# PimLb/POMDP_PBVI_Exploration

Hardware: AMD Instinct MI355X
Metric: alpha-vector backups/sec (higher is better)
Workload: dtype f32

## Files before the change

pomdp_pbvi_exploration_amd/csrc/backup_kernels.h:

```cpp
#pragma once
#include "pbvi_common.h"

namespace pbvi {

template <typename T>
struct ModelView {
    int S, S_pad, A, O, R;
    const int32_t* rs;
    const T* rto;
    const T* er;
    const uint8_t* sup;
};

__host__ __device__ __forceinline__ int64_t push_row_index(int o, int a, int b, int A, int B) {
#ifdef PBVI_PUSH_ORDER_OAB
    return ((int64_t)o * A + a) * B + b;
#else
    return ((int64_t)o * B + b) * A + a;
#endif
}

template <typename T>
struct SlabView {
    const T* slabs;
// ... 48 lines not shown
                             int k_tiles, uint8_t* need, hipStream_t st);

template <typename T>
hipError_t launch_dead(const T* bel, int ldb, int B, ModelView<T> mv,
                       const unsigned long long* nzBw ,
                       int k_tiles, uint8_t* dead, int32_t* btl ,
                       int32_t* btc , int* dead_count ,
                       hipStream_t st, const uint8_t* rowflags = nullptr ,
                       const int32_t* perm = nullptr );

template <typename T>
hipError_t launch_push_project(const T* bel, int ldb, int B, ModelView<T> mv, const int32_t* in_ptr,
                               const int32_t* in_src, double gamma, const T* amax, T* bp, int ldp, double* mag,
                               hipStream_t st, uint8_t* nzP = nullptr );
template <typename T>
hipError_t launch_rdot(const T* bel, int ldb, int B, ModelView<T> mv, const int32_t* btl, const int32_t* btc, double* rd,
                       hipStream_t st);

template <typename T>
hipError_t launch_argmax(SlabView<T> sv, int V, int G, int B, const uint8_t* dead, double tol_rel, double tol_abs,
                         const int* chain_steps ,
                         int flag_all, int32_t* best_v, double* best_score, double* err, int32_t* queue, int* qcount,
                         hipStream_t st, double tol_extra = 0.0 ,
                         int split = 0 );

template <typename T>
hipError_t launch_fold_chunk(SlabView<T> sv, int B, int G, int Vc, int V, int v0, int tail_cols, T* dst, int64_t ldd,
                             const int* chain, int* chain_max, hipStream_t st);

struct RefineWork {
    int32_t* items_v = nullptr;
    int32_t* items_slot = nullptr;
    double* scores = nullptr;
    int32_t* slot_entry = nullptr;
    int32_t* slot_n = nullptr;
    int32_t* tiles = nullptr;
    unsigned long long* emax = nullptr;
    int32_t* eidx = nullptr;
    double* ib_val = nullptr;
    int32_t* ib_idx = nullptr;
    int* cnt = nullptr;
    int32_t* q2_entry = nullptr;
    int32_t* q2_n = nullptr;
    int32_t* q2_cand = nullptr;
    double* q2_part = nullptr;
    int* q2_done = nullptr;
    int q2_cap = 0;
// ... 6 lines not shown
    uint8_t* nzW = nullptr;
    int* klistW = nullptr;
    int* kcountW = nullptr;
    const int32_t* in_ptr = nullptr;
    const int32_t* in_src = nullptr;
    const float* gam = nullptr;
    int ldg = 0;
    double l1_rel = 0.0;
};

template <typename T, typename TS>
hipError_t launch_refine(bool proj, SlabView<TS> sv, int V, int G, int max_entries, const int32_t* queue,
                         const int* qcount, const T* bel, int ldb, const T* alpha, int lda, ModelView<T> mv,
                         double gamma, const int32_t* btl, const int32_t* btc ,
                         const uint8_t* nzG ,
                         int32_t* best_v, double* best_score, double* err, int* cand_total ,
                         RefineWork work, hipStream_t st);

template <typename T, typename TS>
hipError_t launch_refine_scan(bool proj, SlabView<TS> sv, int V, int G, int max_entries, const int32_t* queue,
                              const int* qcount, const T* bel, int ldb, const T* alpha, int lda, ModelView<T> mv,
                              double gamma, const int32_t* btl, const int32_t* btc, const uint8_t* nzG, int32_t* best_v,
                              double* best_score, double* err, int* cand_total, RefineWork work, int* counts_host,
                              hipStream_t st);
template <typename T>
hipError_t launch_refine_deferred(bool proj, int V, int G, const T* bel, int ldb, const T* alpha, int lda, ModelView<T> mv,
                                  double gamma, int32_t* best_v, double* best_score, double* err, RefineWork work,
                                  int h_items, int h_slots, hipStream_t st);

template <typename T>
hipError_t launch_belief_tiles(const T* bel, int ldb, int B, int S, int k_tiles, int32_t* btl, int32_t* btc,
                               hipStream_t st);

template <typename T>
hipError_t launch_tail_rows(ModelView<T> mv, T* gam , int64_t row0 , int ldg, hipStream_t st,
                            const int32_t* ctile = nullptr);
template <typename T>
hipError_t launch_action(int B, ModelView<T> mv, SlabView<T> sv, int64_t rd_col0, double tol_rel, const int* chain_steps,
                         const double* best_score, const double* err, double* rdot, double* rdot_err, int32_t* action,
                         int32_t* aqueue, int* aqcount, hipStream_t st, double tol_extra = 0.0,
                         uint8_t* acand = nullptr ,
                         int split = 0 );
constexpr int ACTION_SPLIT = 8;
template <typename T>
hipError_t launch_refine_action(const T* bel, int ldb, int B, const T* alpha, int lda, ModelView<T> mv, double gamma,
                                const int32_t* btl, const int32_t* btc, const int32_t* aqueue, const int* aqcount,
                                const double* rdot, const double* rdot_err, const int32_t* best_v,
// ... 38 lines not shown
```

pomdp_pbvi_exploration_amd/csrc/backup_kernels.hip:

```cpp
#include "backup_kernels.h"

#include <cstdlib>
#include <limits>

namespace pbvi {

__device__ __forceinline__ double wave_sum(double v) {
#pragma unroll
    for (int off = 32; off > 0; off >>= 1) v += __shfl_xor(v, off, 64);
    return v;
}

__device__ __forceinline__ double block_sum(double v, double* sh) {
    v = wave_sum(v);
    const int lane = threadIdx.x & 63, wid = threadIdx.x >> 6;
    __syncthreads();
    if (lane == 0) sh[wid] = v;
    __syncthreads();
    return ((sh[0] + sh[1]) + sh[2]) + sh[3];
}

struct TileList {
    const int32_t* list;
    int count;
// ... 556 lines not shown
    return hipGetLastError();
}

template <typename T>
hipError_t launch_dead(const T* bel, int ldb, int B, ModelView<T> mv, const unsigned long long* nzBw, int k_tiles, uint8_t* dead,
                       int32_t* btl, int32_t* btc, int* dead_count, hipStream_t st, const uint8_t* rowflags,
                       const int32_t* perm) {
    if (B <= 0) return hipSuccess;
    const size_t lds = (size_t)((k_tiles + 7) & ~7) + (size_t)((k_tiles + 63) / 64) * 8;
    hipLaunchKernelGGL(k_dead<T>, dim3(B), dim3(256), lds, st, bel, ldb, mv, nzBw, k_tiles, dead, btl, btc,
                       dead_count, rowflags, perm);
    return hipGetLastError();
}

__device__ __forceinline__ double score_window(double tol_rel, const int* chain_steps, int split) {
    const double u24 = 5.9604644775390625e-08;
    double tr = tol_rel;
    if (chain_steps != nullptr && tol_rel < 0.0)
        tr = 8.0 * u24 * (sqrt((double)chain_steps[0] * 32.0 * (split ? 3.0 : 1.0)) + 1.0);
    if (split) tr = (tr + 3.1 * 1.52587890625e-05) * (1.0 + 4.8828125e-04);
    return tr;
}

template <typename T>
__global__ void k_argmax(SlabView<T> sv, int V, int G, int B, const uint8_t* __restrict__ dead, double tol_rel,
                         double tol_abs, double tol_extra, const int* __restrict__ chain_steps, int flag_all, int32_t* __restrict__ best_v, double* __restrict__ best_score,
                         double* __restrict__ err, int32_t* __restrict__ queue, int* __restrict__ qcount, int split) {
    const int lane = threadIdx.x & 63;
    const int64_t gw = (int64_t)blockIdx.x * 4 + (threadIdx.x >> 6);
    if (gw >= (int64_t)B * G) return;
    const int b = (int)(gw / G), g = (int)(gw % G);
    if (dead != nullptr && dead[gw]) {
        if (lane == 0) {
            best_v[gw] = 0;
            best_score[gw] = 0.0;
            err[gw] = 0.0;
        }
        return;
    }
    T m = -std::numeric_limits<T>::infinity(), m2 = -std::numeric_limits<T>::infinity();
    int idx = 0x7fffffff;
    bool vec4 = false;
    if constexpr (sizeof(T) == 4) vec4 = sv.nchunks != nullptr && (sv.push || (V & 3) == 0) && (sv.ldc & 3) == 0;
    if (vec4) {
        typedef float F4 __attribute__((ext_vector_type(4)));
        const int64_t row = sv.push ? sv.push_row(b, g) : (int64_t)b;
        const int64_t col0 = sv.push ? 0 : (int64_t)g * V;
        const float* rowp = (const float*)sv.slabs + row * sv.ldc + col0;
        const int tm = (int)(row >> 8);
        for (int c00 = lane * 4; c00 < V; c00 += 1024) {
            int n[4], fb[4];
            F4 acc[4];
#pragma unroll
            for (int j = 0; j < 4; ++j) {
                const int c0 = c00 + 256 * j;
                const int64_t pair = ((col0 + c0) >> 8) * sv.tiles_m + tm;
                n[j] = c0 < V ? sv.nchunks[pair] : 0;
                fb[j] = (c0 < V && sv.first_block != nullptr) ? sv.first_block[pair] : 0;
            }
#pragma unroll
            for (int j = 0; j < 4; ++j) {
                const F4 zero = {0.f, 0.f, 0.f, 0.f};
                acc[j] = zero;
                if (n[j] > 0) acc[j] = acc[j] + *(const F4*)(rowp + c00 + 256 * j);
            }
#pragma unroll
            for (int j = 0; j < 4; ++j) {
                if (n[j] <= 1) continue;
                if (sv.first_block != nullptr) {
                    const float* x = (const float*)sv.slabs + sv.slab_stride + (int64_t)(fb[j] + 1) * (256 * 256) +
                                     (row & 255) * 256 + ((col0 + c00 + 256 * j) & 255);
                    for (int z = 1; z < n[j]; ++z, x += 256 * 256) acc[j] = acc[j] + *(const F4*)x;
                } else {
                    for (int z = 1; z < n[j]; ++z) acc[j] = acc[j] + *(const F4*)(rowp + c00 + 256 * j + (int64_t)z * sv.slab_stride);
                }
            }
#pragma unroll
            for (int j = 0; j < 4; ++j) {
                const int c0 = c00 + 256 * j;
                if (c0 >= V) break;
#pragma unroll
                for (int i = 0; i < 4; ++i) {
                    const T sc = (T)acc[j][i];
                    const int v = c0 + i;
                    if (v >= V) break;
                    if (sc > m || idx == 0x7fffffff) {
                        m2 = (idx == 0x7fffffff) ? m2 : m;
                        m = sc;
                        idx = v;
                    } else if (sc > m2) {
                        m2 = sc;
                    }
                }
            }
        }
    } else
    for (int v0 = lane; v0 < V; v0 += 256) {
        T sc4[4];
#pragma unroll
        for (int j = 0; j < 4; ++j) {
            const int v = v0 + 64 * j;
            sc4[j] = v < V ? sv.score(b, g, V, v) : T(0);
        }
#pragma unroll
        for (int j = 0; j < 4; ++j) {
            const int v = v0 + 64 * j;
            if (v >= V) break;
            const T sc = sc4[j];
            if (sc > m || idx == 0x7fffffff) {
                m2 = (idx == 0x7fffffff) ? m2 : m;
                m = sc;
                idx = v;
            } else if (sc > m2) {
                m2 = sc;
            }
        }
    }
#pragma unroll
    for (int off = 32; off > 0; off >>= 1) {
        const T om = __shfl_xor(m, off, 64), om2 = __shfl_xor(m2, off, 64);
        const int oi = __shfl_xor(idx, off, 64);
        const T lo = om < m ? om : m;
        T n2 = m2 > om2 ? m2 : om2;
        if (oi != 0x7fffffff && idx != 0x7fffffff) n2 = lo > n2 ? lo : n2;
        if (om > m || (om == m && oi < idx)) {
            m = om;
            idx = oi;
        }
        m2 = n2;
    }
    double E = 0.0;
    int push = 0;
    if (queue != nullptr) {
        const double mag = fmax(fabs((double)m), fabs(sv.magnitude(b, g, G, V)));
        const double tr = score_window(tol_rel, chain_steps, split) + (sv.push ? 2.0 * 5.9604644775390625e-08 : 0.0);
        E = (tr + tol_extra) * mag + tol_abs;
        push = (flag_all || (double)m2 >= (double)m - 2.0 * E) ? 1 : 0;
    }
    if (lane == 0) {
        best_v[gw] = idx;
        best_score[gw] = (double)m;
        err[gw] = E;
        if (push) {
            const int slot = atomicAdd(qcount, 1);
            queue[slot] = (int32_t)gw;
        }
    }
}

template <typename T>
hipError_t launch_argmax(SlabView<T> sv, int V, int G, int B, const uint8_t* dead, double tol_rel, double tol_abs,
                         const int* chain_steps, int flag_all, int32_t* best_v, double* best_score, double* err,
                         int32_t* queue, int* qcount, hipStream_t st, double tol_extra, int split) {
    const int64_t rows = (int64_t)B * G;
    if (rows <= 0) return hipSuccess;
    hipLaunchKernelGGL(k_argmax<T>, dim3((unsigned)((rows + 3) / 4)), dim3(256), 0, st, sv, V, G, B, dead, tol_rel,
                       tol_abs, tol_extra, chain_steps, flag_all, best_v, best_score, err, queue, qcount, split);
    return hipGetLastError();
}

template <typename T>
__global__ void k_fold_chunk(SlabView<T> sv, int B, int G, int Vc, int V, int v0, int tail_cols, T* __restrict__ dst,
                             int64_t ldd, const int* __restrict__ chain, int* __restrict__ chain_max) {
    if (chain != nullptr && blockIdx.x == 0 && blockIdx.y == 0 && threadIdx.x == 0) {
        const int c = chain[0];
        if (c > chain_max[0]) chain_max[0] = c;
    }
    const int64_t group_cols = (int64_t)G * Vc, n_cols = group_cols + tail_cols;
    const int64_t j0 = ((int64_t)blockIdx.x * 256 + threadIdx.x) * 4;
    if (j0 >= n_cols) return;
    bool vec4 = false;
    if constexpr (sizeof(T) == 4) vec4 = sv.nchunks != nullptr && (Vc & 3) == 0 && (sv.ldc & 3) == 0 && j0 + 3 < group_cols;
    auto out_col = [&](int64_t j) -> int64_t {
        if (j >= group_cols) return (int64_t)G * V + (j - group_cols);
        const int64_t g = j / Vc;
        return g * V + v0 + (j - g * Vc);
    };
    const int64_t d0 = out_col(j0);
    for (int b = blockIdx.y; b < B; b += gridDim.y) {
        T* drow = dst + (int64_t)b * ldd;
// ... 72 lines not shown
                for (int j = 0; j < 4; ++j) g[j] += (double)rto[ro + s[j]] * (double)arow[rs[ro + s[j]]];
            }
#pragma unroll
            for (int j = 0; j < 4; ++j) acc[j] += w[j] * ((double)brow[s[j]] * (gamma * g[j]));
        } else {
#pragma unroll
            for (int j = 0; j < 4; ++j) {
                const bool in = s[j] < mv.S;
                acc[j] += (in ? w[j] : 0.0) * ((double)brow[s[j]] * (double)arow[in ? s[j] : 0]);
            }
        }
    }
    return wave_sum((acc[0] + acc[1]) + (acc[2] + acc[3]));
}

template <typename T, typename TS, bool PROJ, bool L1 >
__global__ void k_refine(SlabView<TS> sv, int V, int G, const int32_t* __restrict__ queue,
                         const int* __restrict__ qcount,
                         const T* __restrict__ bel, int ldb, const T* __restrict__ alpha, int lda,
                         ModelView<T> mv, double gamma, const int32_t* __restrict__ btl, const int32_t* __restrict__ btc,
                         const uint8_t* __restrict__ nzG ,
                         int32_t* __restrict__ best_v,
                         double* __restrict__ best_score, double* __restrict__ err, int* __restrict__ cand_total,
                         RefineWork work) {
    __shared__ int cand[256];
    __shared__ int wcount[4];
    __shared__ int ltile[REFINE_LIST_CAP];
    __shared__ int lbase, loverflow;
    __shared__ int sh_slot, sh_base;
    __shared__ double red[4];
    __shared__ double wbest[4];
    __shared__ int widx[4];
    if ((int)blockIdx.x >= *qcount) return;
    const int tid = threadIdx.x, lane = tid & 63, wid = tid >> 6;
    const int e = queue[blockIdx.x];
    const int b = e / G, g = e % G;
    const int a = PROJ ? g / mv.O : 0, o = PROJ ? g % mv.O : 0;
    const double m = best_score[e], E = err[e];
    const double thr = m - 2.0 * E;
    const T* brow = bel + (int64_t)b * ldb;
    const int k_tiles = mv.S_pad >> 5;
    const int32_t* src = btl ? btl + (int64_t)b * k_tiles : nullptr;
    const int n_src = btl ? btc[b] : k_tiles;
    const uint8_t* zg = (PROJ && nzG) ? nzG + (int64_t)g * k_tiles : nullptr;
    if (tid == 0) {
        lbase = 0;
        loverflow = 0;
    }
    __syncthreads();
    for (int i0 = 0; i0 < n_src; i0 += 256) {
        const int i = i0 + tid;
        int t = 0, f = 0;
        if (i < n_src) {
            t = src ? src[i] : i;
            f = zg ? (zg[t] != 0) : 1;
        }
        const unsigned long long mask = __ballot(f);
        if (lane == 0) wcount[wid] = __popcll(mask);
        __syncthreads();
        int off = lbase;
        for (int w = 0; w < wid; ++w) off += wcount[w];
        const int tot = wcount[0] + wcount[1] + wcount[2] + wcount[3];
// ... 27 lines not shown
                    bestval = tot;
                    bestidx = vv;
                }
            }
        } else {
            for (int c = wid; c < ncand; c += 4) {
                const int vv = cand[c];
                const double tot = refine_wave_dot<T, PROJ>(brow, alpha + (int64_t)vv * lda, mv, a, o, gamma, L, n_tiles, lane);
                if (tot > bestval) {
                    bestval = tot;
                    bestidx = vv;
                }
            }
        }
    };
    bool settled = false;
    if (!loverflow) {
        constexpr int L1_CAP = 32;
        constexpr int FAST_CAP = 8;
        __shared__ int c1[L1_CAP];
        __shared__ double s1[L1_CAP];
        __shared__ double l1red[16];
        __shared__ int n1_sh, n2_sh;
        if (tid == 0) n1_sh = 0;
        __syncthreads();
        for (int v0 = 0; v0 < V; v0 += 256) {
            const int v = v0 + tid;
            int flag = 0;
            if (v < V) flag = ((double)sv.score(b, g, V, v) >= thr) ? 1 : 0;
            const unsigned long long mask = __ballot(flag);
            if (lane == 0) wcount[wid] = __popcll(mask);
            __syncthreads();
            int base = n1_sh;
            for (int w = 0; w < wid; ++w) base += wcount[w];
            const int pos = base + __popcll(mask & ((1ull << lane) - 1ull));
            if (flag && pos < L1_CAP) c1[pos] = v;
            __syncthreads();
            if (tid == 0) n1_sh += wcount[0] + wcount[1] + wcount[2] + wcount[3];
            __syncthreads();
        }
        const int n1 = n1_sh;
        constexpr bool l1 = L1 && PROJ && sizeof(T) == 4;
        if (n1 > 0 && n1 <= L1_CAP && (l1 || n1 <= FAST_CAP)) {
            if (tid == 0 && cand_total != nullptr) atomicAdd(cand_total, n1);
            const TileList tl{L, n_tiles};
            int n2 = n1;
            if constexpr (l1) {
                {
                    for (int c0 = 0; c0 < n1; c0 += 4) {
// ... 367 lines not shown
        wi[wid] = idx;
    }
    __syncthreads();
    if (tid == 0) {
        for (int w = 1; w < 4; ++w)
            if (wv[w] > m || (wv[w] == m && wi[w] < idx)) {
                m = wv[w];
                idx = wi[w];
            }
        if (idx != 0x7fffffff) {
            const int e = work.slot_entry[sl];
            best_v[e] = idx;
            best_score[e] = m;
            err[e] = 0.0;
        }
    }
}

template <typename T, typename TS>
hipError_t launch_refine_scan(bool proj, SlabView<TS> sv, int V, int G, int max_entries, const int32_t* queue,
                              const int* qcount, const T* bel, int ldb, const T* alpha, int lda, ModelView<T> mv,
                              double gamma, const int32_t* btl, const int32_t* btc, const uint8_t* nzG, int32_t* best_v,
                              double* best_score, double* err, int* cand_total, RefineWork work, int* counts_host,
                              hipStream_t st) {
    if (max_entries <= 0) return hipSuccess;
    hipError_t e;
    if (work.items_v != nullptr) {
        if ((e = hipMemsetAsync(work.cnt, 0, work.zero_bytes, st)) != hipSuccess) return e;
    }
    if (proj)
    {
        if (work.gam != nullptr && sizeof(T) == 4) {
            hipLaunchKernelGGL((k_refine<T, TS, true, true>), dim3(max_entries), dim3(256), 0, st, sv, V, G, queue, qcount, bel, ldb,
                               alpha, lda, mv, gamma, btl, btc, nzG, best_v, best_score, err, cand_total, work);
            if (work.q2_entry != nullptr)
                hipLaunchKernelGGL((k_refine_split<T, true>), dim3(work.q2_cap < 256 ? work.q2_cap : 256, REFINE_SPLIT), dim3(256), 0,
                                   st, G, bel, ldb, alpha, lda, mv, gamma, btl, btc, nzG, best_v, best_score, err, work);
        } else
            hipLaunchKernelGGL((k_refine<T, TS, true, false>), dim3(max_entries), dim3(256), 0, st, sv, V, G, queue, qcount, bel, ldb,
                               alpha, lda, mv, gamma, btl, btc, nzG, best_v, best_score, err, cand_total, work);
    }
    else
        hipLaunchKernelGGL((k_refine<T, TS, false, false>), dim3(max_entries), dim3(256), 0, st, sv, V, G, queue, qcount, bel,
                           ldb, alpha, lda, mv, gamma, btl, btc, nzG, best_v, best_score, err, cand_total, work);
    if ((e = hipGetLastError()) != hipSuccess) return e;
    if (work.items_v != nullptr && counts_host != nullptr)
        if ((e = hipMemcpyAsync(counts_host, work.cnt, 2 * sizeof(int), hipMemcpyDeviceToHost, st)) != hipSuccess) return e;
    return hipSuccess;
}

template <typename T>
hipError_t launch_refine_deferred(bool proj, int V, int G, const T* bel, int ldb, const T* alpha, int lda, ModelView<T> mv,
                                  double gamma, int32_t* best_v, double* best_score, double* err, RefineWork work,
                                  int h_items, int h_slots, hipStream_t st) {
    hipError_t e;
    if (work.items_v == nullptr) return hipSuccess;
    const int n_items = h_items < work.item_cap ? h_items : work.item_cap;
    const int n_slots = h_slots < work.slot_cap ? h_slots : work.slot_cap;
    const int n_w = n_slots < work.w_slot_cap ? n_slots : work.w_slot_cap;
    if (n_w > 0) {
        dim3 wgrid((mv.S_pad + 255) / 256, n_w);
        if (proj)
            hipLaunchKernelGGL((k_refine_weights<T, true>), wgrid, dim3(256), 0, st, G, bel, ldb, mv, gamma, work);
        else
            hipLaunchKernelGGL((k_refine_weights<T, false>), wgrid, dim3(256), 0, st, G, bel, ldb, mv, gamma, work);
        if ((e = hipGetLastError()) != hipSuccess) return e;
        if ((e = launch_tile_nonzero_f64(work.W, mv.S_pad, n_w, mv.S_pad / 32, work.nzW, st)) != hipSuccess) return e;
// ... 18 lines not shown
        const int blocks = 2048;
        if (proj)
            hipLaunchKernelGGL((k_refine_items<T, true>), dim3(blocks), dim3(256), 0, st, G, bel, ldb, alpha, lda, mv,
                               gamma, work);
        else
            hipLaunchKernelGGL((k_refine_items<T, false>), dim3(blocks), dim3(256), 0, st, G, bel, ldb, alpha, lda, mv,
                               gamma, work);
        if ((e = hipGetLastError()) != hipSuccess) return e;
        hipLaunchKernelGGL(k_refine_first, dim3(1024), dim3(256), 0, st, work);
        if ((e = hipGetLastError()) != hipSuccess) return e;
    }
    if (n_slots > n_w) hipLaunchKernelGGL(k_refine_merge, dim3(64), dim3(256), 0, st, work, best_v, best_score, err);
    return hipGetLastError();
}

template <typename T, typename TS>
hipError_t launch_refine(bool proj, SlabView<TS> sv, int V, int G, int max_entries, const int32_t* queue,
                         const int* qcount, const T* bel, int ldb, const T* alpha, int lda, ModelView<T> mv,
                         double gamma, const int32_t* btl, const int32_t* btc, const uint8_t* nzG, int32_t* best_v,
                         double* best_score, double* err, int* cand_total, RefineWork work, hipStream_t st) {
    if (max_entries <= 0) return hipSuccess;
    int h_cnt[2] = {0, 0};
    hipError_t e = launch_refine_scan<T, TS>(proj, sv, V, G, max_entries, queue, qcount, bel, ldb, alpha, lda, mv, gamma, btl,
                                             btc, nzG, best_v, best_score, err, cand_total, work, h_cnt, st);
    if (e != hipSuccess || work.items_v == nullptr) return e;
    if ((e = hipStreamSynchronize(st)) != hipSuccess) return e;
    return launch_refine_deferred<T>(proj, V, G, bel, ldb, alpha, lda, mv, gamma, best_v, best_score, err, work, h_cnt[0],
                                     h_cnt[1], st);
}

template <typename T>
__global__ void k_tail_rows(ModelView<T> mv, T* __restrict__ gam, int64_t row0, int ldg, const int32_t* __restrict__ ctile) {
    const int s = blockIdx.x * 256 + threadIdx.x;
    const int j = blockIdx.y;
    if (s >= mv.S_pad) return;
    const T e = mv.er[(int64_t)(j % mv.A) * mv.S_pad + s];
    const int64_t row = row0 + j;
    const int64_t at = ctile != nullptr ? (int64_t)ctile[row >> 8] * 256 + (row & 255) : row;
    gam[at * ldg + s] = (j < mv.A) ? e : (e < T(0) ? -e : e);
}

template <typename T>
hipError_t launch_tail_rows(ModelView<T> mv, T* gam, int64_t row0, int ldg, hipStream_t st, const int32_t* ctile) {
    hipLaunchKernelGGL(k_tail_rows<T>, dim3((mv.S_pad + 255) / 256, 2 * mv.A), dim3(256), 0, st, mv, gam, row0, ldg, ctile);
    return hipGetLastError();
}

// ... 630 lines not shown
    const int blocks = (mv.S_pad + 255) / 256;
    if (rto64 != nullptr)
        hipLaunchKernelGGL(k_walk_push<double>, dim3(blocks), dim3(256), 0, st, base, rto64, mv.S, mv.S_pad, mv.O, mv.R,
                           in_ptr, in_src, a, o, unnorm, partial);
    else
        hipLaunchKernelGGL(k_walk_push<T>, dim3(blocks), dim3(256), 0, st, base, mv.rto, mv.S, mv.S_pad, mv.O, mv.R, in_ptr,
                           in_src, a, o, unnorm, partial);
    hipError_t e = hipGetLastError();
    if (e != hipSuccess) return e;
    hipLaunchKernelGGL(k_walk_norm<T>, dim3(blocks), dim3(256), 0, st, unnorm, partial, blocks, mv.S, mv.S_pad, out64,
                       out_store);
    return hipGetLastError();
}

#define PBVI_INST(T)                                                                                                   \
    template hipError_t launch_support<T>(ModelView<T>, uint8_t*, hipStream_t);                                        \
    template hipError_t launch_project<T>(const T*, int, int, ModelView<T>, T, T*, int, const uint8_t*, int,           \
                                          hipStream_t, const uint8_t*, const int*, int, const int32_t*, const int32_t*); \
    template hipError_t launch_tail_rows<T>(ModelView<T>, T*, int64_t, int, hipStream_t, const int32_t*);               \
    template hipError_t launch_dead<T>(const T*, int, int, ModelView<T>, const unsigned long long*, int, uint8_t*, int32_t*, \
                                       int32_t*, int*, hipStream_t, const uint8_t*, const int32_t*);                                                   \
    template hipError_t launch_belief_tiles<T>(const T*, int, int, int, int, int32_t*, int32_t*, hipStream_t);         \
    template hipError_t launch_argmax<T>(SlabView<T>, int, int, int, const uint8_t*, double, double, const int*, int,  \
                                         int32_t*, double*, double*, int32_t*, int*, hipStream_t, double, int);        \
    template hipError_t launch_fold_chunk<T>(SlabView<T>, int, int, int, int, int, int, T*, int64_t, const int*, int*,   \
                                             hipStream_t);                                                             \
    template hipError_t launch_refine<T, T>(bool, SlabView<T>, int, int, int, const int32_t*, const int*, const T*, int, \
                                         const T*, int, ModelView<T>, double, const int32_t*, const int32_t*,          \
                                         const uint8_t*, int32_t*, double*, double*, int*, RefineWork, hipStream_t);   \
    template hipError_t launch_action<T>(int, ModelView<T>, SlabView<T>, int64_t, double, const int*, const double*,   \
                                         const double*, double*, double*, int32_t*, int32_t*, int*, hipStream_t, double, uint8_t*, \
                                         int);                                                                          \
    template hipError_t launch_refine_action<T>(const T*, int, int, const T*, int, ModelView<T>, double,               \
                                                const int32_t*, const int32_t*, const int32_t*, const int*,            \
                                                const double*, const double*, const int32_t*, const double*,           \
                                                const double*, double*, int32_t*, hipStream_t, const uint8_t*);                        \
    template hipError_t launch_assemble<T>(const T*, int, ModelView<T>, double, const int32_t*, const int32_t*,        \
                                           const int32_t*, const int*, int, T*, int, hipStream_t);                     \
    template hipError_t launch_expand_rows<T>(const T*, const int32_t*, T*, int, int, hipStream_t);                    \
    template hipError_t launch_keep<T>(const T*, int, const T*, int, int, int, const double*, const int32_t*,          \
                                       const int32_t*, uint8_t*, hipStream_t);                                         \
    template hipError_t launch_belief_update<T>(const T*, int, int, ModelView<T>, const int32_t*, const int32_t*,      \
                                                const int32_t*, const int32_t*, const int32_t*, double*, double*, T*,  \
                                                int, hipStream_t);                                                     \
    template hipError_t launch_push_project<T>(const T*, int, int, ModelView<T>, const int32_t*, const int32_t*,       \
                                               double, const T*, T*, int, double*, hipStream_t, uint8_t*);                      \
    template hipError_t launch_rdot<T>(const T*, int, int, ModelView<T>, const int32_t*, const int32_t*, double*,      \
                                       hipStream_t);                                                                   \
    template hipError_t launch_walk_step<T>(const double*, ModelView<T>, const double*, const int32_t*, const int32_t*, \
                                            int, int, double*, double*, double*, T*, hipStream_t);                     \
    template hipError_t launch_walk_fused<T>(const double*, const double*, const double*, double*, T*, ModelView<T>,      \
                                             const double*, const int32_t*, const int32_t*, int, int, double*, double*,   \
                                             hipStream_t);                                                               \
    template hipError_t launch_walk_finish<T>(const double*, const double*, ModelView<T>, double*, T*, hipStream_t);     \
    template hipError_t launch_dominated<T>(const T*, int, int, int, int*, hipStream_t);
PBVI_INST(float)
PBVI_INST(double)
#define PBVI_INST_REFINE(T, TS)                                                                                        \
    template hipError_t launch_refine_scan<T, TS>(bool, SlabView<TS>, int, int, int, const int32_t*, const int*, const T*, \
                                                  int, const T*, int, ModelView<T>, double, const int32_t*, const int32_t*, \
                                                  const uint8_t*, int32_t*, double*, double*, int*, RefineWork, int*,   \
                                                  hipStream_t);
PBVI_INST_REFINE(float, float)
PBVI_INST_REFINE(double, double)
PBVI_INST_REFINE(double, float)
template hipError_t launch_refine_deferred<float>(bool, int, int, const float*, int, const float*, int, ModelView<float>, double,
                                                  int32_t*, double*, double*, RefineWork, int, int, hipStream_t);
template hipError_t launch_refine_deferred<double>(bool, int, int, const double*, int, const double*, int, ModelView<double>,
                                                   double, int32_t*, double*, double*, RefineWork, int, int, hipStream_t);
template hipError_t launch_refine<double, float>(bool, SlabView<float>, int, int, int, const int32_t*, const int*, const double*,
                                                 int, const double*, int, ModelView<double>, double, const int32_t*,
                                                 const int32_t*, const uint8_t*, int32_t*, double*, double*, int*, RefineWork,
                                                 hipStream_t);

}
```

pomdp_pbvi_exploration_amd/csrc/engine.hip:

```cpp
#include <algorithm>
#include <cmath>
#include <cstdio>
#include <cstdlib>
#include <cstring>
#include <condition_variable>
#include <mutex>
#include <new>
#include <string>
#include <thread>
#include <unistd.h>
#include <vector>

#include "backup_kernels.h"
#include "split_bf16.h"

namespace pbvi {

static thread_local std::string g_err;
static int g_poison = -1;
static bool poison_enabled() {
    if (g_poison < 0) g_poison = getenv("PBVI_POISON") != nullptr ? 1 : 0;
    return g_poison == 1;
}
void set_error(const std::string& msg) { g_err = msg; }
// ... 578 lines not shown
            out->bytes = bytes_of(4);
            return PBVI_ENOMEM;
        }
        while (lo < hi) {
            const int64_t mid = (lo / 4 + hi / 4 + 1) / 2 * 4;
            if (bytes_of(mid) <= budget) lo = mid;
            else hi = mid - 4;
        }
        const int64_t n = (V + lo - 1) / lo;
        Vc = round_up((V + n - 1) / n, 4);
    }
    out->chunk_rows = Vc;
    out->n_chunks = (V + Vc - 1) / Vc;
    out->bytes = bytes_of(Vc);
    return out->bytes <= budget ? PBVI_OK : PBVI_ENOMEM;
}

struct ScoreIO {
    int32_t* best_v;
    double* best_score;
    double* err;
    int32_t* queue;
    int* qcount;
    const uint8_t* dead;
    const double* prd;
    hipEvent_t join;
    hipStream_t side;
    hipEvent_t* ev;
    bool stats;
    double tol_extra;
    bool allow_split;
};
template <typename TS>
struct ScoreStage {
    SlabView<TS> sv;
    GemmPlan plan;
    double tol_rel;
    const int* chain;
    int64_t rd_col0, extra_row0, f64_pairs;
    bool fused;
    int split;
    int chunks;
};

class EngineBase {
   public:
    virtual ~EngineBase() {}
    virtual int alpha_set(const void* alpha, int64_t V) = 0;
    virtual int alpha_append(const void* alpha, int64_t n) = 0;
    virtual int64_t alpha_count() const = 0;
    virtual int beliefs_set(const void* bel, int64_t B) = 0;
    virtual int backup_run(double gamma, int flags, pbvi_stats_t* st) = 0;
    virtual int backup_fetch(void* out_alpha, int32_t* out_action, int32_t* out_best, uint8_t* out_keep) = 0;
    virtual int device_results(void** d_alpha, int32_t** d_action, uint8_t** d_keep) = 0;
    virtual int64_t unique_count() const = 0;
    virtual int fetch_unique(void* out_rows, int32_t* out_index) = 0;
    virtual int fetch_compact(void* out_rows, int32_t* out_index, int32_t* out_action, int32_t* out_best, uint8_t* out_keep) = 0;
    virtual int run_fetch(double gamma, int flags, pbvi_stats_t* st, void* out_rows, int64_t cap_rows, int32_t* out_slot,
                          int32_t* out_index, int32_t* out_action, int32_t* out_best, uint8_t* out_keep, int64_t* n_unique,
                          int64_t* n_slots) = 0;
    virtual int fetch_unique_keys(int32_t* out_keys) = 0;
    virtual int fetch_row_hashes(uint64_t* out) = 0;
    virtual int fetch_exchange(int32_t* out, int64_t per) = 0;
    virtual int assemble_keys(double gamma, int64_t n, const int32_t* keys, void* out_rows) = 0;
    virtual int64_t assemble_keys_store(double gamma, int64_t n, const int32_t* keys, void* out_rows) = 0;
// ... 99 lines not shown
    bool h_perm_valid_ = false;
    bool sorted_ = false;
    const void* gam_pad_ptr_ = nullptr;
    int64_t gam_pad_N_ = -1;
    DevBuf scr_flag_;
    DevBuf rowflags_;
    uint64_t rowflags_ver_ = 0;
    uint64_t nzA_ver_ = 0;
    void* ids_pin_ = nullptr;
    size_t ids_pin_cap_ = 0;
    int* h_flag_ = nullptr;
    void* early_rows_ = nullptr;
    int64_t early_cap_ = 0;
    bool early_used_ = false, early_dma_pending_ = false;
    struct RunFetchDst {
        int32_t *slot = nullptr, *index = nullptr, *action = nullptr, *best = nullptr;
        uint8_t* keep = nullptr;
        bool queued = false;
    } rf_dst_;
    DevBuf e_bv_, e_bs_, e_err_, e_rdot_, e_act_, e_ares_, e_bres_, e_rep_, e_uniq_, e_inv_, e_slotd_, e_cnt_, e_out_, e_slot_;
    hipEvent_t ev_early_[2] = {nullptr, nullptr};
    hipEvent_t ev_ids_ = nullptr;
    hipEvent_t ev_nzA_ = nullptr;
    DevBuf nzBw_;
    DevBuf nzB_, nzA_, klist_, kcount_, nchunks_, need_, skws_;
    DevBuf dense_, nzD_, nzAlpha_, prod_, klistD_, kcountD_, nchunksD_;
    int64_t rows_pad_s_ = 0, dense_pairs_ = 0;
    std::vector<int> h_kcountD_;
    int* kc_pin_ = nullptr;
    size_t kc_pin_cap_ = 0;
    hipStream_t stream2_ = nullptr;
    hipStream_t stream3_ = nullptr;
    hipEvent_t ev_fork_ = nullptr, ev_join_ = nullptr, ev_lists_ = nullptr, ev_xr_[2] = {nullptr, nullptr};
    GemmPlan plan_ = {};
    hipEvent_t ev_[9] = {};
    hipEvent_t ev_pg_[2] = {};
    bool have_result_ = false, res_sorted_ = false;
    int64_t res_B_ = 0;
    int screen_mode_ = 1;
    int split_mode_ = 1;
    bool split_supported_ = false;
    int fuse_project_ = 1;
    double irr_frac_ = 0.0;
    DevBuf irr_;
    DevBuf mat_, vlist_;
    DevBuf ctile_;
// ... 7 lines not shown
    int64_t dead_pairs_ = 0, dead_count_ = 0;
    int* rf_counts_ = nullptr;
    bool last_deferred_nothing_ = false;
    bool owns_streams_ = true;
    EngineT<float>* screen_ = nullptr;
    std::vector<int32_t> h_reach_ref_;
    std::vector<double> h_rto_ref_, h_er_ref_;
    uint64_t alpha_ver_ = 1, bel_ver_ = 1;
    uint64_t screen_alpha_seen_ = 0, screen_bel_seen_ = 0;

    ~EngineT() override {
        (void)hipSetDevice(device_);
        if (screen_) {
            (void)hipStreamSynchronize(stream_);
            delete screen_;
            screen_ = nullptr;
        }
        DevBuf* all[] = {&rs_, &rto_, &er_, &sup_, &alpha_buf_, &alpha_small_, &bel_, &belsp_, &gam_, &slabs_, &best_v_, &best_score_, &err_,
                         &dead_, &queue_, &counters_, &rdot_, &action_, &aqueue_, &out_, &keep_, &bv2_, &bs2_,
                         &err2_, &queue2_, &prune_cnt_, &nzB_, &nzA_, &klist_, &kcount_, &nchunks_, &need_, &skws_, &stage_, &keys_, &perm_,
                         &action_res_, &best_res_, &rep_, &uniq_, &inv_, &slot_, &out_full_, &btl_, &btc_, &val_exact_, &store_[0], &store_[1], &ids_, &in_ptr_, &in_src_, &bu_act_, &bu_obs_,
                         &bu_unnorm_, &bu_mass_, &bu_out_, &bu_row_, &walk64_, &rto64_, &bp_, &nzP_, &pmag_, &prd_, &keys_tmp_, &keys_act_, &keys_best_, &keys_rows_, &rf_v_, &rf_slot_, &rf_sc_, &rf_entry_, &rf_n_, &rf_tiles_,
                         &snz_, &sbtl_, &sbtc_, &vmax_bk_, &rf_ibv_, &rf_ibi_, &rf_cnt_, &rf_W_, &rf_Cx_, &rf_nzW_, &rf_klW_, &rf_kcW_,
                         &dense_, &nzD_, &nzAlpha_, &prod_, &klistD_, &kcountD_, &nchunksD_, &mat_, &vlist_, &irr_, &rowflags_, &nzBw_, &scr_flag_, &ctile_, &acand_, &rf_q2_, &rf_q2p_, &rf_q2d_, &e_bv_, &e_bs_, &e_err_, &e_rdot_, &e_act_, &e_ares_, &e_bres_, &e_rep_, &e_uniq_, &e_inv_, &e_slotd_, &e_cnt_, &e_out_, &e_slot_, &scores_, &chain_max_};
        static const bool dbg = getenv("PBVI_DEBUG") != nullptr;
        auto chk = [&](hipError_t e, const char* what) {
            if (e != hipSuccess && dbg) fprintf(stderr, "[pbvi] engine teardown: %s: %s\n", what, hipGetErrorString(e));
        };
        for (auto& e : walk_ev_)
            if (e) chk(hipEventDestroy(e), "hipEventDestroy(walk)");
        for (DevBuf* b : all) b->release();
        for (auto& e : tile_ev_)
            if (e) chk(hipEventDestroy(e), "hipEventDestroy(tile)");
        if (host_stage_) chk(hipHostFree(host_stage_), "hipHostFree(stage)");
        if (ids_pin_) chk(hipHostFree(ids_pin_), "hipHostFree(ids)");
        if (h_flag_) chk(hipHostFree(h_flag_), "hipHostFree(flag)");
        if (kc_pin_) chk(hipHostFree(kc_pin_), "hipHostFree(kcount)");
        for (hipEvent_t& ev : ev_early_)
            if (ev) chk(hipEventDestroy(ev), "hipEventDestroy(early)");
        if (ev_ids_) chk(hipEventDestroy(ev_ids_), "hipEventDestroy(ids)");
        if (ev_nzA_) chk(hipEventDestroy(ev_nzA_), "hipEventDestroy(nzA)");
        for (auto& e : ev_)
            if (e) chk(hipEventDestroy(e), "hipEventDestroy(ev)");
        for (auto& e : ev_pg_)
            if (e) chk(hipEventDestroy(e), "hipEventDestroy(ev_pg)");
        if (ev_fork_) chk(hipEventDestroy(ev_fork_), "hipEventDestroy(fork)");
        if (ev_join_) chk(hipEventDestroy(ev_join_), "hipEventDestroy(join)");
// ... 1839 lines not shown
                }
            }
            HIPCHK(launch_project<T>(alpha_.as<T>(), S_pad_, (int)Vt, mv, (T)gamma, gam_.as<T>(), S_pad_, need, k_tiles, stream_,
                                     fused ? mat_.as<uint8_t>() : nullptr, fused && R_ == 1 ? vlist_.as<int>() : nullptr,
                                     fused && R_ == 1 ? (int)h_vlist_.size() : 0,
                                     fused && R_ > 1 ? irr_.as<int32_t>() : nullptr, ctile));
        }
        HIPCHK(launch_tail_rows<T>(mv, gam_.as<T>(), (int64_t)AO * Vt, S_pad_, stream_, ctile));
        HIPCHK(hipEventRecord(io.ev[1], stream_));
        int split = want_split;
        if ((rc = score_gemm(gam_.as<T>(), N, nzB_.as<uint8_t>(), AO, (int)V_, &sv, nullptr, 0, nullptr, io.side, fused, &split)))
            return rc;
        out->split = split;
        out->fused = fused != nullptr;
    }
    HIPCHK(hipEventRecord(io.ev[2], stream_));
    HIPCHK(hipStreamWaitEvent(stream_, io.join, 0));
    out->plan = plan_;
    const int k_chunk = kF32 ? plan_.chunk_len * GEMM_BK : S_pad_;
    out->tol_rel = tie_window(k_chunk);
    out->chain = chain_steps();
    out->rd_col0 = (int64_t)AO * Vt;
    out->f64_pairs = f64_pairs_;
    HIPCHK(launch_argmax<T>(sv, (int)V_, AO, (int)B_, io.dead, out->tol_rel, 0.0, out->chain, 0, io.best_v, io.best_score,
                            io.err, io.queue, io.qcount, stream_, io.tol_extra, out->split));
    HIPCHK(hipEventRecord(io.ev[3], stream_));
    out->sv = sv;
    return PBVI_OK;
}

template <typename T>
int EngineT<T>::ensure_exact(DevBuf& b, size_t bytes) {
    if (bytes > b.cap && b.p != nullptr) {
        HIPCHK(hipStreamSynchronize(stream_));
        bytes_ -= (int64_t)b.cap;
        b.release();
    }
    return b.ensure(bytes, &bytes_);
}

template <typename T>
int EngineT<T>::stage_scores_tiled(double gamma, const ScoreIO& io, int want_split, int64_t Vc, int64_t n_chunks,
                                   ScoreStage<T>* out) {
    int rc;
    const int AO = A_ * O_;
    const int64_t Vt = V_ + 1, N = (int64_t)AO * Vt + 2 * A_;
    const ModelView<T> mv = view();
    const int k_tiles = S_pad_ / GEMM_BK;
// ... 250 lines not shown
            dead_ver_ = bel_ver_;
            dead_pairs_ = pairs;
            dead_count_ = -1;
        }
    }
    if (use_push) {
        if ((rc = prd_.ensure((size_t)B_ * A_ * sizeof(double), &bytes_))) return rc;
        HIPCHK(launch_rdot<T>(bel_.as<T>(), S_pad_, (int)B_, mv, windows ? btl_.as<int32_t>() : nullptr,
                              windows ? btc_.as<int32_t>() : nullptr, prd_.as<double>(), side));
    }
    const bool early_wanted = windows && early_rows_ != nullptr && !(flags & PBVI_BELIEF_DOMINANCE) && early_cap_ >= B_ && !no_side;
    if (early_wanted) {
        if ((rc = e_cnt_.ensure(4 * sizeof(int), &bytes_))) return rc;
        HIPCHK(hipMemsetAsync(e_cnt_.p, 0, 4 * sizeof(int), side));
    }
    HIPCHK(hipEventRecord(ev_join_, side));

    ScoreIO io;
    io.best_v = best_v_.as<int32_t>();
    io.best_score = best_score_.as<double>();
    io.err = err_.as<double>();
    io.queue = windows ? queue_.as<int32_t>() : nullptr;
    io.qcount = qcount;
    io.dead = windows ? dead_.as<uint8_t>() : nullptr;
    io.prd = use_push ? prd_.as<double>() : nullptr;
    io.join = ev_join_;
    io.side = lists;
    io.ev = ev_;
    io.stats = st != nullptr;
    io.tol_extra = screened ? 4.0 * 5.9604644775390625e-08 : 0.0;
    io.allow_split = !screened;
    if (windows && !use_push && scorer.tiling_mode_ != 0) {
        RefineWork reserve;
        if ((rc = refine_work(pairs, V_, &reserve))) return rc;
    }
    ScoreStage<TS> sc;
    if ((rc = scorer.stage_scores(gamma, use_push, io, &sc))) return rc;
    const SlabView<TS>& sv = sc.sv;
    const GemmPlan plan = sc.plan;
    bool xr_pending = false;
    if (use_push && !screened) {
        if ((rc = vmax_bk_.ensure((size_t)B_ * sizeof(double), &bytes_))) return rc;
        hipStream_t xs = no_side ? stream_ : stream2_;
        if (xs != stream_) {
            HIPCHK(hipEventRecord(ev_xr_[0], stream_));
            HIPCHK(hipStreamWaitEvent(xs, ev_xr_[0], 0));
// ... 71 lines not shown
        early_used_ = true;
    }
    RefineWork work;
    bool speculate = false;
    if (windows) {
        if ((rc = refine_work(pairs, V_, &work))) return rc;
        if constexpr (kF32 && !screened) {
            static const bool no_l1 = getenv("PBVI_NO_L1_SCREEN") != nullptr;
            if (!no_l1 && !use_push && !sc.fused && sc.chunks <= 1 && mode_ == PBVI_SPARSE) {
                work.gam = (const float*)gam_.p;
                work.ldg = S_pad_;
                work.l1_rel = (double)(R_ + 4) * 5.9604644775390625e-08;
            }
        }
        rf_counts_ = pinned_flag();
        if (!rf_counts_) FAIL(PBVI_ENOMEM, "backup_run: pinned flag");
        rf_counts_ += 24;
        rf_counts_[0] = rf_counts_[1] = 0;
        static const bool no_spec = getenv("PBVI_NO_SPECULATION") != nullptr;
        speculate = !no_spec && last_deferred_nothing_ && work.items_v != nullptr && !(flags & PBVI_BELIEF_DOMINANCE);
        HIPCHK((launch_refine_scan<T, TS>(true, sv, (int)V_, AO, (int)pairs, queue_.as<int32_t>(), qcount, bel_.as<T>(), S_pad_,
                                          alpha_.as<T>(), S_pad_, mv, gamma, btl_.as<int32_t>(), btc_.as<int32_t>(),
                                          nzB_.as<uint8_t>(), best_v_.as<int32_t>(), best_score_.as<double>(), err_.as<double>(),
                                          counters_.as<int>() + 4, work, rf_counts_, stream_)));
        if (!speculate && work.items_v != nullptr) {
            HIPCHK(hipStreamSynchronize(stream_));
            last_deferred_nothing_ = rf_counts_[0] == 0 && rf_counts_[1] == 0;
            HIPCHK(launch_refine_deferred<T>(true, (int)V_, AO, bel_.as<T>(), S_pad_, alpha_.as<T>(), S_pad_, mv, gamma,
                                             best_v_.as<int32_t>(), best_score_.as<double>(), err_.as<double>(), work,
                                             rf_counts_[0], rf_counts_[1], stream_));
        }
    }
    if (early_used_ && early_dma_pending_) {
        HIPCHK(hipEventSynchronize(ev_early_[0]));
        const int np = h_flag_[8];
        if (np > 0)
            HIPCHK(hipMemcpyAsync(early_rows_, e_out_.p, (size_t)np * S_ * sizeof(T), hipMemcpyDeviceToHost, stream2_));
        HIPCHK(hipEventRecord(ev_early_[1], stream2_));
        early_dma_pending_ = false;
    }
    if (h_kcount != nullptr)
        HIPCHK(hipMemcpyAsync(kc_pin_, scorer.kcount_.p, n_kcount * sizeof(int), hipMemcpyDeviceToHost, stream_));
    HIPCHK(hipEventRecord(ev_[4], stream_));
    const int32_t* perm = sorted_ ? perm_.as<int32_t>() : nullptr;
    int* ucount = counters_.as<int>() + 3;
    int h_cnt[8] = {0, 0, 0, 0, 0, 0, 0, 0};
    auto later_stages = [&]() -> int {
// ... 691 lines not shown
```

Before: 649,000.

## Hand off top-two candidates from argmax to refine to skip rescans

The argmax kernel gains a handoff variant that tracks the top three scores per row. When exactly two candidates fall within the tolerance window, it records the runner-up index so the refine kernel can seed its candidate list directly instead of rescanning all V scores. The variant also batches queue atomics per block using shared-memory prefix counts and runs 8 waves per block. The cost is extra register and shuffle work in argmax and an additional per-pair buffer.

```diff
diff --git a/pomdp_pbvi_exploration_amd/csrc/backup_kernels.h b/pomdp_pbvi_exploration_amd/csrc/backup_kernels.h
--- a/pomdp_pbvi_exploration_amd/csrc/backup_kernels.h
+++ b/pomdp_pbvi_exploration_amd/csrc/backup_kernels.h
@@ -94,7 +94,8 @@
                          const int* chain_steps ,
                          int flag_all, int32_t* best_v, double* best_score, double* err, int32_t* queue, int* qcount,
                          hipStream_t st, double tol_extra = 0.0 ,
-                         int split = 0 );
+                         int split = 0 ,
+                         int32_t* cand2 = nullptr );
 
 template <typename T>
 hipError_t launch_fold_chunk(SlabView<T> sv, int B, int G, int Vc, int V, int v0, int tail_cols, T* dst, int64_t ldd,
@@ -147,7 +148,7 @@
                               const int* qcount, const T* bel, int ldb, const T* alpha, int lda, ModelView<T> mv,
                               double gamma, const int32_t* btl, const int32_t* btc, const uint8_t* nzG, int32_t* best_v,
                               double* best_score, double* err, int* cand_total, RefineWork work, int* counts_host,
-                              hipStream_t st);
+                              hipStream_t st, const int32_t* cand2 = nullptr );
 template <typename T>
 hipError_t launch_refine_deferred(bool proj, int V, int G, const T* bel, int ldb, const T* alpha, int lda, ModelView<T> mv,
                                   double gamma, int32_t* best_v, double* best_score, double* err, RefineWork work,
diff --git a/pomdp_pbvi_exploration_amd/csrc/backup_kernels.hip b/pomdp_pbvi_exploration_amd/csrc/backup_kernels.hip
--- a/pomdp_pbvi_exploration_amd/csrc/backup_kernels.hip
+++ b/pomdp_pbvi_exploration_amd/csrc/backup_kernels.hip
@@ -602,24 +602,52 @@
     return tr;
 }
 
-template <typename T>
+constexpr int ARGMAX_WAVES = 4, ARGMAX_WAVES_HANDOFF = 8;
+template <typename T, bool HANDOFF>
 __global__ void k_argmax(SlabView<T> sv, int V, int G, int B, const uint8_t* __restrict__ dead, double tol_rel,
                          double tol_abs, double tol_extra, const int* __restrict__ chain_steps, int flag_all, int32_t* __restrict__ best_v, double* __restrict__ best_score,
-                         double* __restrict__ err, int32_t* __restrict__ queue, int* __restrict__ qcount, int split) {
+                         double* __restrict__ err, int32_t* __restrict__ queue, int* __restrict__ qcount, int split,
+                         int32_t* __restrict__ cand2) {
+    constexpr int WAVES = HANDOFF ? ARGMAX_WAVES_HANDOFF : ARGMAX_WAVES;
+    __shared__ int push_w[ARGMAX_WAVES_HANDOFF];
+    __shared__ int slot0;
     const int lane = threadIdx.x & 63;
-    const int64_t gw = (int64_t)blockIdx.x * 4 + (threadIdx.x >> 6);
-    if (gw >= (int64_t)B * G) return;
-    const int b = (int)(gw / G), g = (int)(gw % G);
-    if (dead != nullptr && dead[gw]) {
+    const int64_t gw = (int64_t)blockIdx.x * WAVES + (threadIdx.x >> 6);
+    bool live = gw < (int64_t)B * G;
+    if (!HANDOFF && !live) return;
+    const int b = live ? (int)(gw / G) : 0, g = live ? (int)(gw % G) : 0;
+    if (live && dead != nullptr && dead[gw]) {
         if (lane == 0) {
             best_v[gw] = 0;
             best_score[gw] = 0.0;
             err[gw] = 0.0;
         }
-        return;
+        if (!HANDOFF) return;
+        live = false;
     }
     T m = -std::numeric_limits<T>::infinity(), m2 = -std::numeric_limits<T>::infinity();
-    int idx = 0x7fffffff;
+    T m3 = -std::numeric_limits<T>::infinity();
+    int idx = 0x7fffffff, idx2 = 0x7fffffff;
+    auto take = [&](T sc, int v) {
+        if (sc > m || idx == 0x7fffffff) {
+            if (HANDOFF && idx != 0x7fffffff) {
+                m3 = m2;
+                idx2 = idx;
+            }
+            m2 = (idx == 0x7fffffff) ? m2 : m;
+            m = sc;
+            idx = v;
+        } else if (sc > m2) {
+            if (HANDOFF) {
+                m3 = m2;
+                idx2 = v;
+            }
+            m2 = sc;
+        } else if (HANDOFF && sc > m3) {
+            m3 = sc;
+        }
+    };
+    const int V_scan = live ? V : 0;
     bool vec4 = false;
     if constexpr (sizeof(T) == 4) vec4 = sv.nchunks != nullptr && (sv.push || (V & 3) == 0) && (sv.ldc & 3) == 0;
     if (vec4) {
@@ -628,7 +656,7 @@
         const int64_t col0 = sv.push ? 0 : (int64_t)g * V;
         const float* rowp = (const float*)sv.slabs + row * sv.ldc + col0;
         const int tm = (int)(row >> 8);
-        for (int c00 = lane * 4; c00 < V; c00 += 1024) {
+        for (int c00 = lane * 4; c00 < V_scan; c00 += 1024) {
             int n[4], fb[4];
             F4 acc[4];
 #pragma unroll
@@ -664,18 +692,12 @@
                     const T sc = (T)acc[j][i];
                     const int v = c0 + i;
                     if (v >= V) break;
-                    if (sc > m || idx == 0x7fffffff) {
-                        m2 = (idx == 0x7fffffff) ? m2 : m;
-                        m = sc;
-                        idx = v;
-                    } else if (sc > m2) {
-                        m2 = sc;
-                    }
+                    take(sc, v);
                 }
             }
         }
     } else
-    for (int v0 = lane; v0 < V; v0 += 256) {
+    for (int v0 = lane; v0 < V_scan; v0 += 256) {
         T sc4[4];
 #pragma unroll
         for (int j = 0; j < 4; ++j) {
@@ -686,14 +708,7 @@
         for (int j = 0; j < 4; ++j) {
             const int v = v0 + 64 * j;
             if (v >= V) break;
-            const T sc = sc4[j];
-            if (sc > m || idx == 0x7fffffff) {
-                m2 = (idx == 0x7fffffff) ? m2 : m;
-                m = sc;
-                idx = v;
-            } else if (sc > m2) {
-                m2 = sc;
-            }
+            take(sc4[j], v);
         }
     }
 #pragma unroll
@@ -703,7 +718,21 @@
         const T lo = om < m ? om : m;
         T n2 = m2 > om2 ? m2 : om2;
         if (oi != 0x7fffffff && idx != 0x7fffffff) n2 = lo > n2 ? lo : n2;
-        if (om > m || (om == m && oi < idx)) {
+        const bool other = om > m || (om == m && oi < idx);
+        if constexpr (HANDOFF) {
+            const T om3 = __shfl_xor(m3, off, 64);
+            const int oi2 = __shfl_xor(idx2, off, 64);
+            const T w2 = other ? om2 : m2, w3 = other ? om3 : m3, l1 = other ? m : om, l2 = other ? m2 : om2;
+            const int wi2 = other ? oi2 : idx2, li1 = other ? idx : oi;
+            if (li1 != 0x7fffffff && l1 > w2) {
+                idx2 = li1;
+                m3 = w2 > l2 ? w2 : l2;
+            } else {
+                idx2 = wi2;
+                m3 = (li1 != 0x7fffffff && l1 > w3) ? l1 : w3;
+            }
+        }
+        if (other) {
             m = om;
             idx = oi;
         }
@@ -711,19 +740,46 @@
     }
     double E = 0.0;
     int push = 0;
-    if (queue != nullptr) {
+    if (queue != nullptr && live) {
         const double mag = fmax(fabs((double)m), fabs(sv.magnitude(b, g, G, V)));
         const double tr = score_window(tol_rel, chain_steps, split) + (sv.push ? 2.0 * 5.9604644775390625e-08 : 0.0);
         E = (tr + tol_extra) * mag + tol_abs;
         push = (flag_all || (double)m2 >= (double)m - 2.0 * E) ? 1 : 0;
     }
-    if (lane == 0) {
-        best_v[gw] = idx;
-        best_score[gw] = (double)m;
-        err[gw] = E;
-        if (push) {
-            const int slot = atomicAdd(qcount, 1);
+    if constexpr (!HANDOFF) {
+        if (lane == 0) {
+            best_v[gw] = idx;
+            best_score[gw] = (double)m;
+            err[gw] = E;
+            if (push) {
+                const int slot = atomicAdd(qcount, 1);
+                queue[slot] = (int32_t)gw;
+            }
+        }
+    } else {
+        const int wid = threadIdx.x >> 6;
+        if (lane == 0) {
+            if (live) {
+                best_v[gw] = idx;
+                best_score[gw] = (double)m;
+                err[gw] = E;
+            }
+            push_w[wid] = push;
+        }
+        __syncthreads();
+        if (threadIdx.x == 0) {
+            int n = 0;
+            for (int w = 0; w < WAVES; ++w) n += push_w[w];
+            slot0 = n > 0 ? atomicAdd(qcount, n) : 0;
+        }
+        __syncthreads();
+        if (lane == 0 && push) {
+            int slot = slot0;
+            for (int w = 0; w < wid; ++w) slot += push_w[w];
             queue[slot] = (int32_t)gw;
+            const double thr = (double)m - 2.0 * E;
+            const bool two = !flag_all && idx2 != 0x7fffffff && (double)m2 >= thr && !((double)m3 >= thr);
+            cand2[gw] = two ? idx2 : -1;
         }
     }
 }
@@ -731,11 +787,17 @@
 template <typename T>
 hipError_t launch_argmax(SlabView<T> sv, int V, int G, int B, const uint8_t* dead, double tol_rel, double tol_abs,
                          const int* chain_steps, int flag_all, int32_t* best_v, double* best_score, double* err,
-                         int32_t* queue, int* qcount, hipStream_t st, double tol_extra, int split) {
+                         int32_t* queue, int* qcount, hipStream_t st, double tol_extra, int split, int32_t* cand2) {
     const int64_t rows = (int64_t)B * G;
     if (rows <= 0) return hipSuccess;
-    hipLaunchKernelGGL(k_argmax<T>, dim3((unsigned)((rows + 3) / 4)), dim3(256), 0, st, sv, V, G, B, dead, tol_rel,
-                       tol_abs, tol_extra, chain_steps, flag_all, best_v, best_score, err, queue, qcount, split);
+    if (cand2 != nullptr && queue != nullptr) {
+        constexpr int W = ARGMAX_WAVES_HANDOFF;
+        hipLaunchKernelGGL((k_argmax<T, true>), dim3((unsigned)((rows + W - 1) / W)), dim3(64 * W), 0, st, sv, V, G, B, dead,
+                           tol_rel, tol_abs, tol_extra, chain_steps, flag_all, best_v, best_score, err, queue, qcount, split, cand2);
+        return hipGetLastError();
+    }
+    hipLaunchKernelGGL((k_argmax<T, false>), dim3((unsigned)((rows + 3) / 4)), dim3(256), 0, st, sv, V, G, B, dead, tol_rel,
+                       tol_abs, tol_extra, chain_steps, flag_all, best_v, best_score, err, queue, qcount, split, nullptr);
     return hipGetLastError();
 }
 
@@ -854,7 +916,7 @@
                          const uint8_t* __restrict__ nzG ,
                          int32_t* __restrict__ best_v,
                          double* __restrict__ best_score, double* __restrict__ err, int* __restrict__ cand_total,
-                         RefineWork work) {
+                         RefineWork work, const int32_t* __restrict__ cand2 ) {
     __shared__ int cand[256];
     __shared__ int wcount[4];
     __shared__ int ltile[REFINE_LIST_CAP];
@@ -870,6 +932,8 @@
     const int a = PROJ ? g / mv.O : 0, o = PROJ ? g % mv.O : 0;
     const double m = best_score[e], E = err[e];
     const double thr = m - 2.0 * E;
+    const int hand2 = cand2 != nullptr ? cand2[e] : -1;
+    const int hand1 = hand2 >= 0 ? best_v[e] : -1;
     const T* brow = bel + (int64_t)b * ldb;
     const int k_tiles = mv.S_pad >> 5;
     const int32_t* src = btl ? btl + (int64_t)b * k_tiles : nullptr;
@@ -943,9 +1007,15 @@
         __shared__ double s1[L1_CAP];
         __shared__ double l1red[16];
         __shared__ int n1_sh, n2_sh;
-        if (tid == 0) n1_sh = 0;
+        if (tid == 0) {
+            n1_sh = hand2 >= 0 ? 2 : 0;
+            if (hand2 >= 0) {
+                c1[0] = hand1 < hand2 ? hand1 : hand2;
+                c1[1] = hand1 < hand2 ? hand2 : hand1;
+            }
+        }
         __syncthreads();
-        for (int v0 = 0; v0 < V; v0 += 256) {
+        for (int v0 = 0; v0 < V && hand2 < 0; v0 += 256) {
             const int v = v0 + tid;
             int flag = 0;
             if (v < V) flag = ((double)sv.score(b, g, V, v) >= thr) ? 1 : 0;
@@ -1359,7 +1429,7 @@
                               const int* qcount, const T* bel, int ldb, const T* alpha, int lda, ModelView<T> mv,
                               double gamma, const int32_t* btl, const int32_t* btc, const uint8_t* nzG, int32_t* best_v,
                               double* best_score, double* err, int* cand_total, RefineWork work, int* counts_host,
-                              hipStream_t st) {
+                              hipStream_t st, const int32_t* cand2) {
     if (max_entries <= 0) return hipSuccess;
     hipError_t e;
     if (work.items_v != nullptr) {
@@ -1369,17 +1439,17 @@
     {
         if (work.gam != nullptr && sizeof(T) == 4) {
             hipLaunchKernelGGL((k_refine<T, TS, true, true>), dim3(max_entries), dim3(256), 0, st, sv, V, G, queue, qcount, bel, ldb,
-                               alpha, lda, mv, gamma, btl, btc, nzG, best_v, best_score, err, cand_total, work);
+                               alpha, lda, mv, gamma, btl, btc, nzG, best_v, best_score, err, cand_total, work, cand2);
             if (work.q2_entry != nullptr)
                 hipLaunchKernelGGL((k_refine_split<T, true>), dim3(work.q2_cap < 256 ? work.q2_cap : 256, REFINE_SPLIT), dim3(256), 0,
                                    st, G, bel, ldb, alpha, lda, mv, gamma, btl, btc, nzG, best_v, best_score, err, work);
         } else
             hipLaunchKernelGGL((k_refine<T, TS, true, false>), dim3(max_entries), dim3(256), 0, st, sv, V, G, queue, qcount, bel, ldb,
-                               alpha, lda, mv, gamma, btl, btc, nzG, best_v, best_score, err, cand_total, work);
+                               alpha, lda, mv, gamma, btl, btc, nzG, best_v, best_score, err, cand_total, work, cand2);
     }
     else
         hipLaunchKernelGGL((k_refine<T, TS, false, false>), dim3(max_entries), dim3(256), 0, st, sv, V, G, queue, qcount, bel,
-                           ldb, alpha, lda, mv, gamma, btl, btc, nzG, best_v, best_score, err, cand_total, work);
+                           ldb, alpha, lda, mv, gamma, btl, btc, nzG, best_v, best_score, err, cand_total, work, cand2);
     if ((e = hipGetLastError()) != hipSuccess) return e;
     if (work.items_v != nullptr && counts_host != nullptr)
         if ((e = hipMemcpyAsync(counts_host, work.cnt, 2 * sizeof(int), hipMemcpyDeviceToHost, st)) != hipSuccess) return e;
@@ -1444,7 +1514,7 @@
     if (max_entries <= 0) return hipSuccess;
     int h_cnt[2] = {0, 0};
     hipError_t e = launch_refine_scan<T, TS>(proj, sv, V, G, max_entries, queue, qcount, bel, ldb, alpha, lda, mv, gamma, btl,
-                                             btc, nzG, best_v, best_score, err, cand_total, work, h_cnt, st);
+                                             btc, nzG, best_v, best_score, err, cand_total, work, h_cnt, st, nullptr);
     if (e != hipSuccess || work.items_v == nullptr) return e;
     if ((e = hipStreamSynchronize(st)) != hipSuccess) return e;
     return launch_refine_deferred<T>(proj, V, G, bel, ldb, alpha, lda, mv, gamma, best_v, best_score, err, work, h_cnt[0],
@@ -2121,7 +2191,7 @@
                                        int32_t*, int*, hipStream_t, const uint8_t*, const int32_t*);                                                   \
     template hipError_t launch_belief_tiles<T>(const T*, int, int, int, int, int32_t*, int32_t*, hipStream_t);         \
     template hipError_t launch_argmax<T>(SlabView<T>, int, int, int, const uint8_t*, double, double, const int*, int,  \
-                                         int32_t*, double*, double*, int32_t*, int*, hipStream_t, double, int);        \
+                                         int32_t*, double*, double*, int32_t*, int*, hipStream_t, double, int, int32_t*); \
     template hipError_t launch_fold_chunk<T>(SlabView<T>, int, int, int, int, int, int, T*, int64_t, const int*, int*,   \
                                              hipStream_t);                                                             \
     template hipError_t launch_refine<T, T>(bool, SlabView<T>, int, int, int, const int32_t*, const int*, const T*, int, \
@@ -2159,7 +2229,7 @@
     template hipError_t launch_refine_scan<T, TS>(bool, SlabView<TS>, int, int, int, const int32_t*, const int*, const T*, \
                                                   int, const T*, int, ModelView<T>, double, const int32_t*, const int32_t*, \
                                                   const uint8_t*, int32_t*, double*, double*, int*, RefineWork, int*,   \
-                                                  hipStream_t);
+                                                  hipStream_t, const int32_t*);
 PBVI_INST_REFINE(float, float)
 PBVI_INST_REFINE(double, double)
 PBVI_INST_REFINE(double, float)
diff --git a/pomdp_pbvi_exploration_amd/csrc/engine.hip b/pomdp_pbvi_exploration_amd/csrc/engine.hip
--- a/pomdp_pbvi_exploration_amd/csrc/engine.hip
+++ b/pomdp_pbvi_exploration_amd/csrc/engine.hip
@@ -624,6 +624,7 @@
     double* err;
     int32_t* queue;
     int* qcount;
+    int32_t* cand2 = nullptr;
     const uint8_t* dead;
     const double* prd;
     hipEvent_t join;
@@ -643,6 +644,7 @@
     bool fused;
     int split;
     int chunks;
+    int32_t* cand2 = nullptr;
 };
 
 class EngineBase {
@@ -788,6 +790,7 @@
     hipEvent_t ev_early_[2] = {nullptr, nullptr};
     hipEvent_t ev_ids_ = nullptr;
     hipEvent_t ev_nzA_ = nullptr;
+    DevBuf cand2_;
     DevBuf nzBw_;
     DevBuf nzB_, nzA_, klist_, kcount_, nchunks_, need_, skws_;
     DevBuf dense_, nzD_, nzAlpha_, prod_, klistD_, kcountD_, nchunksD_;
@@ -841,7 +844,7 @@
                          &action_res_, &best_res_, &rep_, &uniq_, &inv_, &slot_, &out_full_, &btl_, &btc_, &val_exact_, &store_[0], &store_[1], &ids_, &in_ptr_, &in_src_, &bu_act_, &bu_obs_,
                          &bu_unnorm_, &bu_mass_, &bu_out_, &bu_row_, &walk64_, &rto64_, &bp_, &nzP_, &pmag_, &prd_, &keys_tmp_, &keys_act_, &keys_best_, &keys_rows_, &rf_v_, &rf_slot_, &rf_sc_, &rf_entry_, &rf_n_, &rf_tiles_,
                          &snz_, &sbtl_, &sbtc_, &vmax_bk_, &rf_ibv_, &rf_ibi_, &rf_cnt_, &rf_W_, &rf_Cx_, &rf_nzW_, &rf_klW_, &rf_kcW_,
-                         &dense_, &nzD_, &nzAlpha_, &prod_, &klistD_, &kcountD_, &nchunksD_, &mat_, &vlist_, &irr_, &rowflags_, &nzBw_, &scr_flag_, &ctile_, &acand_, &rf_q2_, &rf_q2p_, &rf_q2d_, &e_bv_, &e_bs_, &e_err_, &e_rdot_, &e_act_, &e_ares_, &e_bres_, &e_rep_, &e_uniq_, &e_inv_, &e_slotd_, &e_cnt_, &e_out_, &e_slot_, &scores_, &chain_max_};
+                         &dense_, &nzD_, &nzAlpha_, &prod_, &klistD_, &kcountD_, &nchunksD_, &mat_, &vlist_, &irr_, &rowflags_, &nzBw_, &cand2_, &scr_flag_, &ctile_, &acand_, &rf_q2_, &rf_q2p_, &rf_q2d_, &e_bv_, &e_bs_, &e_err_, &e_rdot_, &e_act_, &e_ares_, &e_bres_, &e_rep_, &e_uniq_, &e_inv_, &e_slotd_, &e_cnt_, &e_out_, &e_slot_, &scores_, &chain_max_};
         static const bool dbg = getenv("PBVI_DEBUG") != nullptr;
         auto chk = [&](hipError_t e, const char* what) {
             if (e != hipSuccess && dbg) fprintf(stderr, "[pbvi] engine teardown: %s: %s\n", what, hipGetErrorString(e));
@@ -2727,8 +2730,9 @@
     out->chain = chain_steps();
     out->rd_col0 = (int64_t)AO * Vt;
     out->f64_pairs = f64_pairs_;
+    out->cand2 = use_push ? nullptr : io.cand2;
     HIPCHK(launch_argmax<T>(sv, (int)V_, AO, (int)B_, io.dead, out->tol_rel, 0.0, out->chain, 0, io.best_v, io.best_score,
-                            io.err, io.queue, io.qcount, stream_, io.tol_extra, out->split));
+                            io.err, io.queue, io.qcount, stream_, io.tol_extra, out->split, out->cand2));
     HIPCHK(hipEventRecord(io.ev[3], stream_));
     out->sv = sv;
     return PBVI_OK;
@@ -3025,6 +3029,11 @@
     io.err = err_.as<double>();
     io.queue = windows ? queue_.as<int32_t>() : nullptr;
     io.qcount = qcount;
+    static const bool tail_legacy = getenv("PBVI_TAIL_LEGACY") != nullptr;
+    if (windows && !tail_legacy) {
+        if ((rc = cand2_.ensure((size_t)pairs * sizeof(int32_t), &bytes_))) return rc;
+        io.cand2 = cand2_.as<int32_t>();
+    }
     io.dead = windows ? dead_.as<uint8_t>() : nullptr;
     io.prd = use_push ? prd_.as<double>() : nullptr;
     io.join = ev_join_;
@@ -3142,7 +3151,7 @@
         HIPCHK((launch_refine_scan<T, TS>(true, sv, (int)V_, AO, (int)pairs, queue_.as<int32_t>(), qcount, bel_.as<T>(), S_pad_,
                                           alpha_.as<T>(), S_pad_, mv, gamma, btl_.as<int32_t>(), btc_.as<int32_t>(),
                                           nzB_.as<uint8_t>(), best_v_.as<int32_t>(), best_score_.as<double>(), err_.as<double>(),
-                                          counters_.as<int>() + 4, work, rf_counts_, stream_)));
+                                          counters_.as<int>() + 4, work, rf_counts_, stream_, sc.cand2)));
         if (!speculate && work.items_v != nullptr) {
             HIPCHK(hipStreamSynchronize(stream_));
             last_deferred_nothing_ = rf_counts_[0] == 0 && rf_counts_[1] == 0;
```

New measurement: 669,400 (median of 6 runs). 3.1% higher.
